# leekwoon/nav-gym

Hardware: AMD Instinct MI355X
Metric: env steps/sec (whole node), 4096 envs x 1081-beam lidar (higher is better)
Workload: dtype f32

## Files before the change

nav-gym_amd/csrc/kernels_step.hpp:

```cpp

struct StepShared {
    double rp[3];
    double old_rp[3];
    double act[2];
    float lx, ly, lth;
    int steps_now;
    double cT, sT;
    int i0, j0;
    int nseg, ndisc;
    int rescan;
    int respawn;
    float t1;
    float r_all;
    unsigned long long step_key;
    unsigned long long rescan_key;
    int next_chunk;
    int park_count, park_next;
    int pair_done;
    int term;
    int vote;
    double lin_step;
    float march_lim;
    double wave_ratio[kMaxWaves];
};
#ifndef NAVSIM_STEP_CONSTS_LDS
#define NAVSIM_STEP_CONSTS_LDS 1
#endif
#ifndef NAVSIM_STEP_VOTE_LDS
#define NAVSIM_STEP_VOTE_LDS 1
#endif
__device__ __forceinline__ double scan_lin_step(const navsim_config& c, const StepShared& sh) {
    if constexpr (NAVSIM_STEP_CONSTS_LDS) return sh.lin_step;
    else return nv::linspace_step(c);
}
__device__ __forceinline__ float scan_march_limit(const navsim_config& c, const StepShared& sh) {
    if constexpr (NAVSIM_STEP_CONSTS_LDS) return sh.march_lim;
    else return march_limit(c.map_h, c.map_w, c.range_max, c.resolution);
}
__device__ __forceinline__ void step_consts_publish(const navsim_config& c, StepShared& sh, int which) {
    const double num = which ? c.range_max : c.angle_last - c.angle_min;
    const double den = which ? c.resolution : (double)(c.n_beams - 1);
    const double q = num / den;
    if (which) {
        const float full = (float)((long long)c.map_h * c.map_w);
        const float lim = (float)(floor(q) + 4.0);
        sh.march_lim = lim < full ? lim : full;
    } else {
        sh.lin_step = (c.n_beams > 1) ? q : 0.0;
    }
}
struct PedShared {
    double *ax, *ay, *avx, *avy;
    float (*seg)[4];
    float (*disc)[2];
    float* info;
};
__host__ __device__ inline size_t ped_lds_bytes(int N) { return (size_t)144 * N + 32; }
__host__ __device__ inline size_t ped_pair_bytes(int N) { return ((size_t)(N * (N - 1) / 2 + N) * sizeof(double2) + 15) & ~(size_t)15; }
__device__ __forceinline__ PedShared ped_lds_carve(char* base, int N) {
    PedShared ps;
    double* d = (double*)base;
    ps.ax = d; ps.ay = d + (N + 1); ps.avx = d + 2 * (N + 1); ps.avy = d + 3 * (N + 1);
    float* f = (float*)(d + 4 * (N + 1));
    ps.seg = (float(*)[4])f;
    ps.disc = (float(*)[2])(f + 16 * N);
    ps.info = f + 20 * N;
    return ps;
}
struct Prims { const float (*seg)[4]; const float (*disc)[2]; float* info; };

template <int BLOCK>
__device__ __forceinline__ void finish_beams(const navsim_config& c, const StepShared& sh, const Prims pr,
                                             const double* __restrict__ tab, const float2* __restrict__ dir,
                                             const float* __restrict__ rng, float* __restrict__ rng_rw,
                                             const float* __restrict__ thr, const float* __restrict__ dthr,
                                             float* __restrict__ obs_row, int n_hist, float noise_std,
                                             uint64_t noise_key, uint64_t genv, int& crash, int& discomfort);

__device__ __forceinline__ void sfm_pair(const navsim_config& c, double xi, double yi, double vxi, double vyi,
                                         double xj, double yj, double vxj, double vyj, double& fx, double& fy) {
    fx = 0.0; fy = 0.0;
    double dxx = xj - xi, dyy = yj - yi;
    double dist = sqrt(dxx * dxx + dyy * dyy);
    if (dist < 1e-9) return;
    double ddx = dxx / dist, ddy = dyy / dist;
    double ivx = c.sfm_lambda * (vxi - vxj) + ddx;
    double ivy = c.sfm_lambda * (vyi - vyj) + ddy;
    double il = sqrt(ivx * ivx + ivy * ivy);
    if (il < 1e-9) return;
    double idx = ivx / il, idy = ivy / il;
    double theta = nv::atan2_(idx * ddy - idy * ddx, idx * ddx + idy * ddy);
    double Bq = c.sfm_gamma * il;
    double a1 = c.sfm_n_prime * Bq * theta;
    double a2 = c.sfm_n * Bq * theta;
    double fv = -nv::exp_neg(-dist / Bq - a1 * a1);
    double sgn = (theta > 0.0) ? 1.0 : ((theta < 0.0) ? -1.0 : 0.0);
    double fa = -sgn * nv::exp_neg(-dist / Bq - a2 * a2);
    fx = fv * idx + fa * (-idy);
    fy = fv * idy + fa * idx;
}

template <typename T>
__device__ __forceinline__ T& at_off32(T* base, int idx) {
    return *(T*)((char*)base + (unsigned)idx * (unsigned)sizeof(T));
}

__device__ __forceinline__ bool beam_dir_fast(double lin, double lth, double ct, double st, double cT, double sT,
                                              float& heading, float& dx, float& dy) {
    const double ang = lin + lth;
    heading = (float)ang;
    if constexpr (nv::kDirTwoSum) {
        const double bb = ang - lin;
        const double eps = (lin - (ang - bb)) + (lth - bb);
        const double delta = ((double)heading - ang) + eps;
        return nv::beam_dir_from_table(ct, st, cT, sT, delta, dx, dy);
    } else {
        const double delta = (double)heading - ang;
        const unsigned mag = (unsigned)__double2hiint(ang) & 0x7FFFFFFFu;
        return nv::beam_dir_from_table(ct, st, cT, sT, delta, dx, dy) & (mag < nv::kDirHi64);
    }
}
__device__ __forceinline__ void beam_dir_k(const navsim_config& c, const double* __restrict__ tab, int k,
                                           double step, double lth, double cT, double sT,
                                           float& dx, float& dy) {
#ifdef NAVSIM_DIAG_CHEAP_DIR
    { float h = (float)c.angle_min + (float)k * (float)step + (float)lth; dx = __cosf(h); dy = __sinf(h); return; }
#endif
    const double last = (c.n_beams == 1) ? c.angle_min : c.angle_last;
    const double lin = (k == c.n_beams - 1) ? last : (double)k * step + c.angle_min;
    float heading = (float)(lin + lth);
    bool fast = false;
    if (tab) {
        const double2 cs = at_off32((const double2*)tab, k);
        fast = beam_dir_fast(lin, lth, cs.x, cs.y, cT, sT, heading, dx, dy);
    }
    if (!fast) nv::beam_dir(heading, dx, dy);
}

template <int RULE, typename Field>
__device__ __forceinline__ void first_probe(const Field& field, int map_h, int map_w, int i0, int j0, float max_range,
                                            float& t1, float& r_all) {
    t1 = 0.0f; r_all = -1.0f;
    if (i0 >= map_w || j0 >= map_h) { r_all = max_range; return; }
    typename Field::raw_t raw0 = field.load(i0, j0);
    if (field.occupied(raw0)) { r_all = 0.0f; return; }
    t1 = march_step<RULE>(field.decode(raw0, i0, j0));
    if (!(t1 < max_range)) r_all = max_range;
}

constexpr float kPrimAllBeams = 1.0e30f;
template <int BLOCK> __device__ __forceinline__ int block_threads() { return BLOCK ? BLOCK : (int)blockDim.x; }
template <int BLOCK>
__device__ __forceinline__ void prim_in_range(int nprim, int nseg, float lx, float ly, float rcull, const Prims pr,
                                              float stepf, float beta0) {
    const float kTwoPiF = 6.2831853f;
    for (int p = (int)threadIdx.x; p < nprim; p += block_threads<BLOCK>()) {
        bool skip;
        float ac = 0.0f, w = 0.0f;
        bool full = (stepf <= 0.0f);
        if (p < nseg) {
            float ux = pr.seg[p][0] - lx, uy = pr.seg[p][1] - ly, vx = pr.seg[p][2] - lx, vy = pr.seg[p][3] - ly;
            skip = sqrtf(ux * ux + uy * uy) - sqrtf((vx - ux) * (vx - ux) + (vy - uy) * (vy - uy)) > rcull;
            float b1 = atan2f(uy, ux), b2 = atan2f(vy, vx);
            float d = b2 - b1;
            d -= kTwoPiF * floorf(d / kTwoPiF + 0.5f);
            ac = b1 + 0.5f * d;
            w = 0.5f * fabsf(d);
            if (fabsf(d) > 3.0f || ux * ux + uy * uy < 1e-6f || vx * vx + vy * vy < 1e-6f) full = true;
        } else {
            float ux = pr.disc[p - nseg][0] - lx, uy = pr.disc[p - nseg][1] - ly;
            float dist = sqrtf(ux * ux + uy * uy);
            skip = dist - nv::kLegRadius > rcull;
            if (dist <= nv::kLegRadius * 1.05f) full = true;
            else { ac = atan2f(uy, ux); w = asinf(fminf(1.0f, nv::kLegRadius / dist)); }
        }
        float rel = ac - beta0;
        rel -= kTwoPiF * floorf(rel / kTwoPiF + 0.5f);
// ... 706 lines not shown
    *peds_before = before;
    __syncthreads();
    return rank;
}

#ifndef NAVSIM_INSTALL_UNROLL
#define NAVSIM_INSTALL_UNROLL 8
#endif
struct StepInstallBig { char* dst; const char* src; size_t bytes; };
struct StepInstall {
    navsim_state stage;
    const float* stage_obs;
    uint8_t* mark;
    const long long* ready;
    uint8_t* late_next;
    const uint8_t* late_prev;
    int lone;
    uint8_t* late;
    StepInstallBig big[5];
};
__device__ __forceinline__ void stage_request(int64_t* stage_episode, uint8_t* mark, int e, int64_t ep) {
    __hip_atomic_store(&stage_episode[e], ep, __ATOMIC_RELAXED, __HIP_MEMORY_SCOPE_AGENT);
    __threadfence();
    atomicOr((unsigned*)(mark + (e & ~3)), 1u << (8 * (e & 3)));
}
__device__ __forceinline__ long long stage_ready(const long long* ready, int e) {
    return __hip_atomic_load(&ready[e], __ATOMIC_ACQUIRE, __HIP_MEMORY_SCOPE_AGENT);
}
__device__ __forceinline__ void install_publish(const StepInstall& in, const navsim_state& live, int e) {
    __syncthreads();
    if (threadIdx.x == 0) {
        __threadfence();
        stage_request(in.stage.episode, in.mark, e, live.episode[e] + 1);
    }
}
template <int BLOCK>
__device__ __forceinline__ void install_arena(const navsim_config& c, const navsim_state& live, const navsim_step_io& io,
                                              const StepInstall& in, const int e, float* __restrict__ obs_row) {
    const int tid = threadIdx.x;
    const bool by_slot = live.map_slot && in.stage.map_slot;
    if (by_slot && tid == 0) {
        const int32_t a = live.map_slot[e], b = in.stage.map_slot[e];
        live.map_slot[e] = b; in.stage.map_slot[e] = a;
    }
    for (int k = 0; k < 5 && !by_slot; ++k) {
        if (!in.big[k].dst) continue;
        const size_t bytes = in.big[k].bytes;
        const char* src = in.big[k].src + (size_t)e * bytes;
        char* dst = in.big[k].dst + (size_t)e * bytes;
        if ((((size_t)(uintptr_t)src | (size_t)(uintptr_t)dst | bytes) & 15) == 0) {
            const size_t n16 = bytes / 16;
            size_t i = tid;
#ifndef NAVSIM_DIAG_INSTALL_NO_BIG
            constexpr int U = NAVSIM_INSTALL_UNROLL;
            for (; i + (U - 1) * BLOCK < n16; i += U * BLOCK) {
                typedef unsigned int u32x4 __attribute__((ext_vector_type(4)));
                u32x4 v[U];
#pragma unroll
                for (int u = 0; u < U; ++u) v[u] = __builtin_nontemporal_load((const u32x4*)src + i + u * BLOCK);
#pragma unroll
                for (int u = 0; u < U; ++u) ((u32x4*)dst)[i + u * BLOCK] = v[u];
            }
            for (; i < n16; i += BLOCK) ((uint4*)dst)[i] = ((const uint4*)src)[i];
#endif
        } else {
            for (size_t i = tid; i < bytes; i += BLOCK) dst[i] = src[i];
        }
    }
    const navsim_state& stage = in.stage;
    const int N = c.max_peds, K = c.n_spawn, P = c.max_waypoints, D = c.n_scan_stack * c.n_beams + NAVSIM_OBS_TAIL;
    const bool peds = c.ped_model != NAVSIM_PED_NONE;
#define NAVSIM_ROW_LOAD(name, dstp, srcp, cnt) \
    const size_t n_##name = ((dstp) && (srcp)) ? (size_t)(cnt) : 0; \
    auto v_##name = (srcp)[tid < (int)n_##name ? (size_t)e * n_##name + tid : 0];
#define NAVSIM_ROW_STORE(name, dstp, srcp) \
    if (tid < (int)n_##name) (dstp)[(size_t)e * n_##name + tid] = v_##name; \
    for (size_t i = (size_t)tid + BLOCK; i < n_##name; i += BLOCK) (dstp)[(size_t)e * n_##name + i] = (srcp)[(size_t)e * n_##name + i];
#define NAVSIM_ROW_SRC(p) ((p) ? (p) : (decltype(p))live.steps)
    NAVSIM_ROW_LOAD(noise, live.scan_noise_std, NAVSIM_ROW_SRC(stage.scan_noise_std), 1)
    NAVSIM_ROW_LOAD(pose, live.robot_pose, NAVSIM_ROW_SRC(stage.robot_pose), 3)
    NAVSIM_ROW_LOAD(goal, live.robot_goal, NAVSIM_ROW_SRC(stage.robot_goal), 2)
    NAVSIM_ROW_LOAD(pact, live.prev_action, NAVSIM_ROW_SRC(stage.prev_action), 2)
    NAVSIM_ROW_LOAD(ppose, live.prev_pose, NAVSIM_ROW_SRC(stage.prev_pose), 3)
    NAVSIM_ROW_LOAD(nhist, live.n_hist, NAVSIM_ROW_SRC(stage.n_hist), 1)
    NAVSIM_ROW_LOAD(steps, live.steps, NAVSIM_ROW_SRC(stage.steps), 1)
    NAVSIM_ROW_LOAD(spose, live.spawn_pose, NAVSIM_ROW_SRC(stage.spawn_pose), (size_t)K * 3)
    NAVSIM_ROW_LOAD(sgoal, live.spawn_goal, NAVSIM_ROW_SRC(stage.spawn_goal), (size_t)K * 2)
    NAVSIM_ROW_LOAD(npeds, peds ? live.n_peds : nullptr, NAVSIM_ROW_SRC(stage.n_peds), 1)
    NAVSIM_ROW_LOAD(ppos, peds ? live.ped_pose : nullptr, NAVSIM_ROW_SRC(stage.ped_pose), (size_t)N * 3)
    NAVSIM_ROW_LOAD(pvel, peds ? live.ped_vel : nullptr, NAVSIM_ROW_SRC(stage.ped_vel), (size_t)N * 2)
    NAVSIM_ROW_LOAD(pyaw, peds ? live.ped_prev_yaw : nullptr, NAVSIM_ROW_SRC(stage.ped_prev_yaw), N)
    NAVSIM_ROW_LOAD(pdist, peds ? live.ped_dist : nullptr, NAVSIM_ROW_SRC(stage.ped_dist), (size_t)N * 3)
    NAVSIM_ROW_LOAD(pvpref, peds ? (double*)live.ped_v_pref : nullptr, NAVSIM_ROW_SRC(stage.ped_v_pref), N)
    NAVSIM_ROW_LOAD(plegs, peds ? (uint8_t*)live.ped_has_legs : nullptr, NAVSIM_ROW_SRC(stage.ped_has_legs), N)
    NAVSIM_ROW_LOAD(pwp, peds ? live.ped_waypoints : nullptr, NAVSIM_ROW_SRC(stage.ped_waypoints), (size_t)N * P * 2)
    NAVSIM_ROW_LOAD(pnwp, peds ? live.ped_n_waypoints : nullptr, NAVSIM_ROW_SRC(stage.ped_n_waypoints), N)
    NAVSIM_ROW_LOAD(phead, peds ? live.ped_wp_head : nullptr, NAVSIM_ROW_SRC(stage.ped_wp_head), N)
    NAVSIM_ROW_LOAD(pgoal, peds ? live.ped_goal : nullptr, NAVSIM_ROW_SRC(stage.ped_goal), (size_t)N * 2)
    NAVSIM_ROW_LOAD(obs, obs_row - (size_t)e * D, in.stage_obs, D)
    NAVSIM_ROW_STORE(noise, live.scan_noise_std, stage.scan_noise_std)
    NAVSIM_ROW_STORE(pose, live.robot_pose, stage.robot_pose)
    NAVSIM_ROW_STORE(goal, live.robot_goal, stage.robot_goal)
    NAVSIM_ROW_STORE(pact, live.prev_action, stage.prev_action)
    NAVSIM_ROW_STORE(ppose, live.prev_pose, stage.prev_pose)
    NAVSIM_ROW_STORE(nhist, live.n_hist, stage.n_hist)
    NAVSIM_ROW_STORE(steps, live.steps, stage.steps)
    NAVSIM_ROW_STORE(spose, (double*)live.spawn_pose, stage.spawn_pose)
    NAVSIM_ROW_STORE(sgoal, (double*)live.spawn_goal, stage.spawn_goal)
    NAVSIM_ROW_STORE(npeds, live.n_peds, stage.n_peds)
    NAVSIM_ROW_STORE(ppos, live.ped_pose, stage.ped_pose)
    NAVSIM_ROW_STORE(pvel, live.ped_vel, stage.ped_vel)
    NAVSIM_ROW_STORE(pyaw, live.ped_prev_yaw, stage.ped_prev_yaw)
    NAVSIM_ROW_STORE(pdist, live.ped_dist, stage.ped_dist)
    NAVSIM_ROW_STORE(pvpref, (double*)live.ped_v_pref, stage.ped_v_pref)
    NAVSIM_ROW_STORE(plegs, (uint8_t*)live.ped_has_legs, stage.ped_has_legs)
    NAVSIM_ROW_STORE(pwp, live.ped_waypoints, stage.ped_waypoints)
    NAVSIM_ROW_STORE(pnwp, live.ped_n_waypoints, stage.ped_n_waypoints)
    NAVSIM_ROW_STORE(phead, live.ped_wp_head, stage.ped_wp_head)
    NAVSIM_ROW_STORE(pgoal, live.ped_goal, stage.ped_goal)
    NAVSIM_ROW_STORE(obs, obs_row - (size_t)e * D, in.stage_obs)
#undef NAVSIM_ROW_LOAD
#undef NAVSIM_ROW_STORE
#undef NAVSIM_ROW_SRC
    if (tid == 0) {
        if (io.achieved_goal) { io.achieved_goal[2 * e] = (float)stage.robot_pose[3 * (size_t)e]; io.achieved_goal[2 * e + 1] = (float)stage.robot_pose[3 * (size_t)e + 1]; }
        if (io.desired_goal) { io.desired_goal[2 * e] = (float)stage.robot_goal[2 * (size_t)e]; io.desired_goal[2 * e + 1] = (float)stage.robot_goal[2 * (size_t)e + 1]; }
        if (live.ped_due) live.ped_due[e] = 0ull;
    }
}

template <int BLOCK, bool PEDS, typename Field, int RULE, int RECT, bool PINL, bool INSTALL = false, bool FEAT = true>
__device__ __forceinline__ void step_arena(const navsim_config& c, const navsim_state& st, const navsim_step_io& io, const int e,
                                           int reset_only, const int peds_done, const uint8_t* __restrict__ reset_mask,
                                           unsigned dyn_lds_bytes, int park_lanes, unsigned rect_lds_offset,
                                           const StepInstall* in = nullptr, const int base_prio = 0) {
    __shared__ StepShared sh;
    extern __shared__ __attribute__((aligned(16))) char dyn_lds_all[];
    char* dyn_lds = dyn_lds_all + (RECT == 2 ? rect_lds_offset : 0u);
    PedShared ps = {};
    if constexpr (PEDS) ps = ped_lds_carve(dyn_lds + ((dyn_lds_bytes + 15u) & ~15u), c.max_peds);
    const Prims prims = {ps.seg, ps.disc, ps.info};
    const int tid = threadIdx.x;
    constexpr int kMarchPrio = (BLOCK == 256 && !PEDS) ? 2 : 0;
    __builtin_amdgcn_s_setprio(3);
    unsigned long long t_begin = 0;
    if (st.arena_cost && tid == 0) t_begin = __builtin_amdgcn_s_memrealtime();
    const int B = c.n_beams, S = c.n_scan_stack, N = c.max_peds, D = S * B + 7;
    const double dt = c.time_step;
    const uint64_t genv = (uint64_t)(c.env_index_base + e);
    const int ms = INSTALL ? map_slot_of(c, st, e) : (c.shared_field ? 0 : e);
    const Field field(st.field, st.field_overflow, ms, c.map_h, c.map_w);
    const uint4* rects = RECT ? (const uint4*)st.rect_table + (size_t)ms * rect_tiles_per_map(c.map_h, c.map_w)
                              : nullptr;
    if constexpr (RECT == 2) {
        const size_t row_bytes = rect_index_row_bytes(c.map_h, c.map_w);
        const uint4* src = (const uint4*)((const char*)st.rect_index + (size_t)ms * row_bytes);
        uint4* tab_lds = (uint4*)dyn_lds_all;
        for (int i = threadIdx.x; i < (int)(row_bytes / 16); i += BLOCK) tab_lds[i] = src[i];
        rects = tab_lds;
    }
    float* obs_row = io.obs + (size_t)e * D;
    const float* obs_prev = io.obs_prev ? io.obs_prev + (size_t)e * D : nullptr;
    double* rp_g = st.robot_pose + 3 * (size_t)e;
    double* goal_g = st.robot_goal + 2 * (size_t)e;
    double* pa_g = st.prev_action + 2 * (size_t)e;
    double* pv_g = st.prev_pose + 3 * (size_t)e;

    constexpr bool kFeat = PEDS || FEAT;
    const bool pending = kFeat && !reset_only && io.reset_mask && io.reset_mask[e] != 0;
    if (pending) {
        reset_only = 1;
        if (tid == 0) {
            io.reward[e] = 0.0; io.done[e] = 0; io.is_success[e] = 0.0f; io.is_crash[e] = 0.0f; io.distance[e] = 0.0;
            if (c.max_episode_steps > 0 && io.truncated) io.truncated[e] = 0;
            if (st.ped_due) st.ped_due[e] = 0ull;
        }
        if (c.defer_reset_scan) return;
        if constexpr (INSTALL && BLOCK >= 256 && RULE == NAVSIM_MARCH_F32) {
            if (in->lone && in->ready) {
                if (tid == 0) {
                    const bool lng = c.regen_min_steps <= 0 || st.done_steps[e] >= c.regen_min_steps;
                    const bool rdy = stage_ready(in->ready, e) == (long long)st.episode[e];
                    sh.respawn = lng ? (rdy ? 3 : 5) : 0;
                    if (!(lng && rdy)) stage_request(in->stage.episode, in->mark, e, st.episode[e] + 1);
                    if (st.counters) {
                        atomicAdd(&st.counters[lng ? (rdy ? NAVSIM_COUNTER_REGEN_SERVED : NAVSIM_COUNTER_REGEN_LATE) : NAVSIM_COUNTER_REGEN_SHORT], 1ull);
                        if (lng && !rdy) atomicAdd(&st.counters[NAVSIM_COUNTER_REGEN_SERVED], 1ull);
                    }
                }
                __syncthreads();
                const int verdict = sh.respawn;
                __syncthreads();
                if (verdict == 3) {
                    install_arena<BLOCK>(c, st, io, *in, e, obs_row);
                    install_publish(*in, st, e);
                    return;
                }
                if (verdict == 5) {
                    regen_lone<Field, BLOCK>(c, st, e);
                    if constexpr (RECT == 2) {
                        const size_t row_bytes = rect_index_row_bytes(c.map_h, c.map_w);
                        const uint4* src = (const uint4*)((const char*)st.rect_index + (size_t)ms * row_bytes);
                        uint4* tab_lds = (uint4*)dyn_lds_all;
                        for (int i = threadIdx.x; i < (int)(row_bytes / 16); i += BLOCK) tab_lds[i] = src[i];
                    }
                }
            }
        }
    }
    if (reset_only && reset_mask && !reset_mask[e]) {
        if (obs_prev && obs_prev != obs_row)
            for (int k = tid; k < D; k += BLOCK) obs_row[k] = obs_prev[k];
        return;
    }

    int n = (!PEDS || c.ped_model == NAVSIM_PED_NONE) ? 0 : st.n_peds[e];
    n = n > N ? N : n;
    const float noise_std = (c.add_scan_noise && st.scan_noise_std) ? st.scan_noise_std[e] : 0.0f;

    NAVSIM_STAMP(0);
    double pp[3] = {0.0, 0.0, 0.0};
    double pvel[2] = {0.0, 0.0};
    const bool is_ped = PEDS && tid < n;
    const size_t pq = (size_t)e * N + (is_ped ? tid : 0);
    const bool ped_advance = PEDS && PINL && !reset_only && !peds_done;
    int ped_head = 0, ped_nw = 1;
    if constexpr (PEDS) {
        if (tid < 64) {
            if (is_ped) {
                pp[0] = st.ped_pose[pq * 3]; pp[1] = st.ped_pose[pq * 3 + 1]; pp[2] = st.ped_pose[pq * 3 + 2];
                pvel[0] = st.ped_vel[pq * 2]; pvel[1] = st.ped_vel[pq * 2 + 1];
            }
            if constexpr (PINL) {
                if (ped_advance) ped_head = ped_stage_wave(c, st, n, tid, is_ped, pq, rp_g, pa_g[0], ps, pp, pvel, ped_nw);
            }
        }
    }
    constexpr int kPhase0Thread = (PEDS && BLOCK > 64) ? 64 : 0;
    const int l0 = tid - kPhase0Thread;
    if (l0 >= 0 && l0 < (NAVSIM_STEP_CONSTS_LDS ? 5 : 3)) {
        const double th_old = rp_g[2];
        double a0 = 0.0, a1 = 0.0;
        if (!reset_only) {
            a0 = io.action[2 * e]; a1 = io.action[2 * e + 1];
            if (c.action_kind == NAVSIM_ACTION_WHEELS) {
                const double wl = a0, wr = a1;
                a0 = c.wheel_radius * (wl + wr) * 0.5;
                a1 = c.wheel_radius * (wr - wl) / c.wheel_track;
            }
            if (c.clamp_action) {
                a0 = a0 < c.linvel_lo ? c.linvel_lo : (a0 > c.linvel_hi ? c.linvel_hi : a0);
                a1 = a1 < c.rotvel_lo ? c.rotvel_lo : (a1 > c.rotvel_hi ? c.rotvel_hi : a1);
            }
            if (c.min_turning_radius > 0.0) {
                double lim = fabs(a1) * c.min_turning_radius;
                if (a0 >= 0.0) a0 = (a0 > lim) ? a0 : lim;
                else           a0 = (a0 < -lim) ? a0 : -lim;
            }
        }
        const double th = th_old + a1 * dt;
        const double th_new = reset_only ? th_old : nv::mod_2pi(th);
        const float lth = (float)th_new;
        const double ang = (l0 == 0) ? th_old : ((l0 == 1) ? th : (double)lth);
        double sn, cs;
        nv::sincos(ang, sn, cs);
        const int w0 = kPhase0Thread & 63;
        const double s0 = __shfl(sn, w0), c0 = __shfl(cs, w0), s1 = __shfl(sn, w0 + 1), c1 = __shfl(cs, w0 + 1);
        const double sT = __shfl(sn, w0 + 2), cT = __shfl(cs, w0 + 2);
        if (NAVSIM_STEP_CONSTS_LDS && l0 >= 3) step_consts_publish(c, sh, l0 - 3);
        if (l0 == 0) {
            sh.old_rp[0] = rp_g[0]; sh.old_rp[1] = rp_g[1]; sh.old_rp[2] = th_old;
            sh.nseg = 0; sh.ndisc = 0; sh.rescan = 0; sh.respawn = 0; sh.term = 0;
            if constexpr (INSTALL) {
                if (pending && !in->lone) {
                    if (in->late) in->late[e] = 0;
                    if (in->late_next) in->late_next[e] = 0;
                    if (in->late_prev && in->late_prev[e]) {
                        sh.respawn = 4;
                        stage_request(in->stage.episode, in->mark, e, st.episode[e] + 1);
                        if (st.counters) atomicAdd(&st.counters[NAVSIM_COUNTER_REGEN_LATE], 1ull);
                    } else if (in->ready) {
                        const bool lng = c.regen_min_steps <= 0 || st.done_steps[e] >= c.regen_min_steps;
                        const bool rdy = stage_ready(in->ready, e) == (long long)st.episode[e];
                        if (lng && rdy) sh.respawn = 3;
                        else {
                            if (lng && in->late) in->late[e] = 1;
                            stage_request(in->stage.episode, in->mark, e, st.episode[e] + 1);
                        }
                        if (st.counters)
                            atomicAdd(&st.counters[lng ? (rdy ? NAVSIM_COUNTER_REGEN_SERVED : NAVSIM_COUNTER_REGEN_LATE) : NAVSIM_COUNTER_REGEN_SHORT], 1ull);
                    }
                }
            }
            if (!reset_only) {
                const int64_t steps_now = st.steps[e] + 1;
                st.steps[e] = steps_now;
                sh.steps_now = (int)steps_now;
                sh.act[0] = a0; sh.act[1] = a1;
                double p[3] = {sh.old_rp[0], sh.old_rp[1], sh.old_rp[2]};
                nv::set_vel_with(p, a0, a1, dt, c.axle_offset, s0, c0, s1, c1, nullptr);
                sh.rp[0] = p[0]; sh.rp[1] = p[1]; sh.rp[2] = p[2];
            } else {
                sh.rp[0] = sh.old_rp[0]; sh.rp[1] = sh.old_rp[1]; sh.rp[2] = sh.old_rp[2];
            }
            sh.lx = (float)sh.rp[0]; sh.ly = (float)sh.rp[1]; sh.lth = (float)sh.rp[2];
            nv::xy_to_ij_f32(sh.lx, sh.ly, c, sh.i0, sh.j0);
            sh.sT = sT; sh.cT = cT;
            first_probe<RULE>(field, c.map_h, c.map_w, sh.i0, sh.j0, (float)((long long)c.map_h * c.map_w), sh.t1, sh.r_all);
            sh.step_key = (unsigned long long)st.episode[e] * 0x100000000ULL +
                          (unsigned long long)(reset_only ? 0 : st.steps[e]) * 2ULL;
            sh.rescan_key = sh.step_key + 1;
            sh.next_chunk = 0; sh.park_count = 0; sh.park_next = 0; sh.pair_done = 0; sh.vote = 0;
        }
    }
    __syncthreads();
    if constexpr (INSTALL) {
        if (pending && sh.respawn == 3) {
            install_arena<BLOCK>(c, st, io, *in, e, obs_row);
            install_publish(*in, st, e);
            return;
        }
        if (pending && sh.respawn == 4) return;
    }

    NAVSIM_STAMP(1);
    if constexpr (PEDS) {
        double2* pair = (double2*)(dyn_lds + ((dyn_lds_bytes + 15u) & ~15u) + ((ped_lds_bytes(N) + 15) & ~(size_t)15));
#ifdef NAVSIM_PAIR_SHARE_ALL
        constexpr int kPairWaves = (BLOCK >= NAVSIM_PAIR_SHARE_MIN_BLOCK) ? 4 : 1;
#else
        constexpr int kPairWaves = (INSTALL && BLOCK >= NAVSIM_PAIR_SHARE_MIN_BLOCK) ? 4 : 1;
#endif
        const bool pair_shared = PINL && kPairWaves > 1 && ped_advance && c.ped_model == NAVSIM_PED_SFM;
        if constexpr (PINL && kPairWaves > 1) {
            if (pair_shared && tid < kPairWaves * 64) ped_pair_share(c, ps, pair, n, tid, kPairWaves, &sh.pair_done);
        }
        if (tid < 64) {
            const int lane = tid;
            if constexpr (PINL) {
                if (ped_advance)
                    ped_advance_wave<Field>(c, st, field, e, n, lane, is_ped, pq, dt, genv, (uint64_t)st.steps[e], ps, pair,
                                            ped_head, ped_nw, pp, pvel, &sh.pair_done, pair_shared ? kPairWaves : 1);
            }
            if (reset_only && is_ped) {
                st.ped_dist[pq * 3] = 0.0; st.ped_dist[pq * 3 + 1] = 0.0; st.ped_dist[pq * 3 + 2] = 0.0;
                st.ped_prev_yaw[pq] = nv::wrap_pi(pp[2]);
            }
            if (is_ped) {
                float dist3[3];
                if (reset_only) { dist3[0] = dist3[1] = dist3[2] = 0.0f; }
                else { dist3[0] = (float)st.ped_dist[pq * 3]; dist3[1] = (float)st.ped_dist[pq * 3 + 1];
                       dist3[2] = (float)st.ped_dist[pq * 3 + 2]; }
                if (st.ped_has_legs[pq] && c.lidar_legs) {
                    float cc[4];
                    nv::leg_centres((float)pp[0], (float)pp[1], (float)pp[2], dist3[0], dist3[1], dist3[2], cc);
                    int q = atomicAdd(&sh.ndisc, 2);
                    ps.disc[q][0] = cc[0]; ps.disc[q][1] = cc[1];
                    ps.disc[q + 1][0] = cc[2]; ps.disc[q + 1][1] = cc[3];
                } else {
                    const double fpx[4] = {0.22, -0.22, -0.22, 0.22};
                    const double fpy[4] = {0.19, 0.19, -0.19, -0.19};
                    double s, cs;
                    nv::sincos(pp[2], s, cs);
                    float vx[4], vy[4];
#pragma unroll
                    for (int v = 0; v < 4; ++v) {
                        vx[v] = (float)((cs * fpx[v] - s * fpy[v]) + pp[0]);
                        vy[v] = (float)((s * fpx[v] + cs * fpy[v]) + pp[1]);
                    }
                    int q = atomicAdd(&sh.nseg, 4);
#pragma unroll
                    for (int v = 0; v < 4; ++v) {
                        int w = (v + 1) & 3;
                        ps.seg[q + v][0] = vx[v]; ps.seg[q + v][1] = vy[v];
                        ps.seg[q + v][2] = vx[w]; ps.seg[q + v][3] = vy[w];
                    }
                }
            }
            wave_lds_sync();
            prims_prepare<64>(c, sh, prims);
        }
    }

    NAVSIM_STAMP(2);
    if (kMarchPrio == 2 || base_prio == 2) __builtin_amdgcn_s_setprio(2);
    else if (base_prio == 1) __builtin_amdgcn_s_setprio(1);
    else __builtin_amdgcn_s_setprio(0);
    int n_hist = reset_only ? 0 : st.n_hist[e];
    int crash = 0, discomfort = 0;
    const uint64_t step_key = sh.step_key;
    float4* park = (float4*)dyn_lds;
    char* scan_lds = dyn_lds + park_lds_bytes(B, park_lanes, PEDS);
    float2* dir_lds = (float2*)scan_lds;
    float* rng_lds = (float*)(scan_lds + sizeof(float2) * (size_t)B);
    scan_beams_pred<BLOCK, Field, PEDS, RULE, RECT>(c, sh, field, rects, st.beam_table, prims, dir_lds, rng_lds, park, park_lanes, st.scan_threshold,
                                                         st.scan_discomfort, obs_row, n_hist, noise_std, step_key, genv, crash, discomfort, false);

    NAVSIM_STAMP(3);
    bool restart_next = false;
    if (!reset_only) {
        vote_flags<BLOCK, PEDS>(sh, crash, discomfort);
        double rmin = 1.0e300;
        if (discomfort && !crash) {
            for (int k = tid; k < B; k += BLOCK)
            {
                double ratio = nv::discomfort_ratio((double)obs_row[(size_t)(S - 1) * B + k],
                                                    st.scan_threshold[k], st.scan_discomfort[k]);
                rmin = ratio < rmin ? ratio : rmin;
            }
            rmin = wave_min_f64(rmin);
            if ((tid & 63) == 0) sh.wave_ratio[tid >> 6] = rmin;
            __syncthreads();
        }
        NAVSIM_STAMP(4);
        if (tid == 0) {
            if (discomfort && !crash)
                for (int w = 1; w < (BLOCK + 63) / 64; ++w) rmin = sh.wave_ratio[w] < rmin ? sh.wave_ratio[w] : rmin;
            double prev_xy[2] = {pv_g[0], pv_g[1]};
            double pose[2] = {sh.rp[0], sh.rp[1]};
            double vel[2] = {pa_g[0], pa_g[1]};
            double goal[2] = {goal_g[0], goal_g[1]};
            nv::RewardOut o = nv::reward_scalar(c, prev_xy, pose, vel, goal, crash != 0, discomfort != 0, rmin);
            if constexpr (kFeat) {
                if (c.max_episode_steps > 0) {
                    const bool trunc = !o.done && sh.steps_now >= c.max_episode_steps;
                    if (io.truncated) io.truncated[e] = (uint8_t)trunc;
                    if (trunc) o.done = 1;
                }
            }
            io.reward[e] = o.reward;
            io.done[e] = (uint8_t)o.done;
            if constexpr (INSTALL) { if (in->late) in->late[e] = 0; if (in->late_next) in->late_next[e] = 0; }
            io.is_success[e] = o.success;
            io.is_crash[e] = o.crash;
            io.distance[e] = o.distance;
            const bool restart = o.done && c.auto_reset != NAVSIM_AUTORESET_NONE && c.n_spawn > 0;
            if (restart && c.auto_reset == NAVSIM_AUTORESET_SAME_STEP) {
                if (kFeat && io.final_obs) {
                    const bool crashed = o.crash != 0.0f;
                    const double tx = crashed ? pv_g[0] : sh.rp[0], ty = crashed ? pv_g[1] : sh.rp[1];
                    const double tyaw = nv::wrap_pi(crashed ? pv_g[2] : sh.rp[2]);
                    float* ft = io.final_obs + (size_t)e * D + (size_t)S * B;
                    ft[0] = (float)pv_g[0]; ft[1] = (float)pv_g[1];
                    ft[2] = (float)tx; ft[3] = (float)ty;
                    ft[4] = (float)pa_g[0]; ft[5] = (float)pa_g[1];
                    ft[6] = (float)tyaw;
                    if (io.final_goals) {
                        float* fg = io.final_goals + 4 * (size_t)e;
                        fg[0] = (float)tx; fg[1] = (float)ty; fg[2] = (float)goal_g[0]; fg[3] = (float)goal_g[1];
                    }
                    sh.term = crashed ? 2 : 1;
                }
                uint64_t h = nv::hash4(c.seed, genv, (uint64_t)st.episode[e], 0x5eedULL);
                int idx = (int)(h % (uint64_t)c.n_spawn);
                const double* sp = st.spawn_pose + ((size_t)e * c.n_spawn + idx) * 3;
                const double* sg = st.spawn_goal + ((size_t)e * c.n_spawn + idx) * 2;
                sh.rp[0] = sp[0]; sh.rp[1] = sp[1]; sh.rp[2] = sp[2];
                goal_g[0] = sg[0]; goal_g[1] = sg[1];
#ifndef NAVSIM_DIAG_NO_DONE_STEPS
                if (st.done_steps) st.done_steps[e] = sh.steps_now;
#endif
                st.episode[e] += 1;
                st.steps[e] = 0;
                sh.rescan_key = (unsigned long long)st.episode[e] * 0x100000000ULL;
                sh.respawn = 1; sh.rescan = c.defer_reset_scan ? 0 : 1;
                if constexpr (INSTALL) if (in->ready) {
                    const bool lng = c.regen_min_steps <= 0 || st.done_steps[e] >= c.regen_min_steps;
                    const bool rdy = stage_ready(in->ready, e) == (long long)st.episode[e];
                    if (lng && rdy) { sh.respawn = 3; sh.rescan = 0; }
                    else if (lng && in->late) in->late[e] = 1;
                    if (st.counters)
                        atomicAdd(&st.counters[lng ? (rdy ? NAVSIM_COUNTER_REGEN_SERVED : NAVSIM_COUNTER_REGEN_LATE) : NAVSIM_COUNTER_REGEN_SHORT], 1ull);
                    if (!(lng && rdy)) stage_request(in->stage.episode, in->mark, e, st.episode[e] + 1);
                }
            } else {
                restart_next = kFeat && restart;
                if (o.crash != 0.0f) {
                    sh.rp[0] = pv_g[0]; sh.rp[1] = pv_g[1]; sh.rp[2] = pv_g[2];
                    sh.rescan = 1;
                }
            }
#ifdef NAVSIM_DIAG_NO_RESCAN
            sh.rescan = 0;
#endif
            if constexpr (!kFeat) {
                if (sh.rescan) {
                    sh.next_chunk = 0; sh.park_count = 0; sh.park_next = 0;
                    sh.lx = (float)sh.rp[0]; sh.ly = (float)sh.rp[1]; sh.lth = (float)sh.rp[2];
                    nv::xy_to_ij_f32(sh.lx, sh.ly, c, sh.i0, sh.j0);
                    nv::sincos((double)sh.lth, sh.sT, sh.cT);
                    first_probe<RULE>(field, c.map_h, c.map_w, sh.i0, sh.j0, (float)((long long)c.map_h * c.map_w), sh.t1, sh.r_all);
                }
            }
        }
        __syncthreads();
        if constexpr (!kFeat) {
            if (sh.rescan) {
                if (sh.respawn) n_hist = 0;
                int c2, d2;
                scan_beams_pred<BLOCK, Field, PEDS, RULE, RECT>(c, sh, field, rects, st.beam_table, prims, dir_lds, rng_lds, park, park_lanes, st.scan_threshold,
                                                                     st.scan_discomfort, obs_row, n_hist, noise_std, sh.rescan_key, genv, c2, d2);
            }
        } else {
            float* final_row = io.final_obs ? io.final_obs + (size_t)e * D : nullptr;
            const int term = sh.term;
            if (term == 1) {
                for (int j = 0; j < S; ++j) {
                    const bool old = j < S - 1 && S - 1 - j <= n_hist;
                    for (int k = tid; k < B; k += BLOCK)
                        final_row[(size_t)j * B + k] = old ? obs_prev[(size_t)(j + 1) * B + k] : obs_row[(size_t)(S - 1) * B + k];
                }
                __syncthreads();
            }
            for (int pass = (term == 2) ? 0 : 1; pass < 2; ++pass) {
                if (pass == 1 && !sh.rescan) break;
                if (tid == 0) {
                    const double* at = (pass == 0) ? pv_g : sh.rp;
                    sh.next_chunk = 0; sh.park_count = 0; sh.park_next = 0;
                    sh.lx = (float)at[0]; sh.ly = (float)at[1]; sh.lth = (float)at[2];
                    nv::xy_to_ij_f32(sh.lx, sh.ly, c, sh.i0, sh.j0);
                    nv::sincos((double)sh.lth, sh.sT, sh.cT);
                    first_probe<RULE>(field, c.map_h, c.map_w, sh.i0, sh.j0, (float)((long long)c.map_h * c.map_w), sh.t1, sh.r_all);
                }
                __syncthreads();
                if (pass == 1 && sh.respawn) n_hist = 0;
                int c2, d2;
                scan_beams_pred<BLOCK, Field, PEDS, RULE, RECT>(c, sh, field, rects, st.beam_table, prims, dir_lds, rng_lds, park, park_lanes, st.scan_threshold,
                                                                     st.scan_discomfort, pass == 0 ? final_row : obs_row, n_hist, noise_std,
                                                                     pass == 0 ? step_key + 1 : sh.rescan_key, genv, c2, d2);
                if (pass == 0) {
                    for (int j = 0; j < S - 1; ++j)
                        if (S - 1 - j <= n_hist)
                            for (int k = tid; k < B; k += BLOCK) final_row[(size_t)j * B + k] = obs_prev[(size_t)(j + 1) * B + k];
                    __syncthreads();
                }
            }
        }
    }

    NAVSIM_STAMP(5);
    if (kMarchPrio != 0 && base_prio < kMarchPrio) {
        if (base_prio == 1) __builtin_amdgcn_s_setprio(1);
        else __builtin_amdgcn_s_setprio(0);
    }
    const bool fresh = reset_only || sh.respawn;
    if (!fresh && obs_prev) {
        for (int j = 0; j < S - 1; ++j)
            if (S - 1 - j <= n_hist)
                for (int k = tid; k < B; k += BLOCK) obs_row[(size_t)j * B + k] = obs_prev[(size_t)(j + 1) * B + k];
    }
    if (tid == 0) {
        float* tail = obs_row + (size_t)S * B;
        double yaw = nv::wrap_pi(sh.rp[2]);
        double pxy0 = fresh ? sh.rp[0] : pv_g[0];
        double pxy1 = fresh ? sh.rp[1] : pv_g[1];
        double v0 = fresh ? 0.0 : pa_g[0], v1 = fresh ? 0.0 : pa_g[1];
        tail[0] = (float)pxy0; tail[1] = (float)pxy1;
        tail[2] = (float)sh.rp[0]; tail[3] = (float)sh.rp[1];
        tail[4] = (float)v0; tail[5] = (float)v1;
        tail[6] = (float)yaw;
        if (io.achieved_goal) { io.achieved_goal[2 * e] = (float)sh.rp[0]; io.achieved_goal[2 * e + 1] = (float)sh.rp[1]; }
        if (io.desired_goal) { io.desired_goal[2 * e] = (float)goal_g[0]; io.desired_goal[2 * e + 1] = (float)goal_g[1]; }
        rp_g[0] = sh.rp[0]; rp_g[1] = sh.rp[1]; rp_g[2] = sh.rp[2];
        if (fresh) { pa_g[0] = 0.0; pa_g[1] = 0.0; st.n_hist[e] = (S - 1 < 1) ? S - 1 : 1; }
        else       { pa_g[0] = sh.act[0]; pa_g[1] = sh.act[1]; st.n_hist[e] = (n_hist + 1 < S - 1) ? n_hist + 1 : S - 1; }
        if (reset_only) st.steps[e] = 0;
        pv_g[0] = sh.rp[0]; pv_g[1] = sh.rp[1]; pv_g[2] = yaw;
        if (restart_next) {
            uint64_t h = nv::hash4(c.seed, genv, (uint64_t)st.episode[e], 0x5eedULL);
            int idx = (int)(h % (uint64_t)c.n_spawn);
            const double* sp = st.spawn_pose + ((size_t)e * c.n_spawn + idx) * 3;
            const double* sg = st.spawn_goal + ((size_t)e * c.n_spawn + idx) * 2;
            rp_g[0] = sp[0]; rp_g[1] = sp[1]; rp_g[2] = sp[2];
            goal_g[0] = sg[0]; goal_g[1] = sg[1];
            if (st.done_steps) st.done_steps[e] = sh.steps_now;
            st.episode[e] += 1;
            st.steps[e] = 0;
            if constexpr (INSTALL) {
                if (in->late_next && in->ready) {
                    const bool lng = c.regen_min_steps <= 0 || sh.steps_now >= c.regen_min_steps;
                    const bool rdy = stage_ready(in->ready, e) == (long long)st.episode[e];
                    in->late_next[e] = (lng && !rdy) ? 1 : 0;
                }
            }
        }
        if (st.arena_cost && !reset_only)
            st.arena_cost[e] = (uint32_t)(__builtin_amdgcn_s_memrealtime() - t_begin);
    }
    NAVSIM_STAMP(6);
    if constexpr (INSTALL) {
        __syncthreads();
        if (sh.respawn == 3) {
            install_arena<BLOCK>(c, st, io, *in, e, obs_row);
            install_publish(*in, st, e);
        }
        NAVSIM_STAMP(7);
    }
}

constexpr int kOrderBuckets = 1024;
struct OrderLds {
    unsigned long long sum;
    unsigned max, pad;
    unsigned wave_tot[16];
    unsigned hist[kOrderBuckets];
};
constexpr size_t kOrderLdsBytes = sizeof(OrderLds);
struct OrderBuckets {
    unsigned long long m;
    float scale;
    __device__ __forceinline__ OrderBuckets(unsigned max, unsigned long long sum, int n) {
        const unsigned long long cap = 4ull * (sum / (unsigned long long)n) + 1ull;
        m = max < cap ? max : cap;
        scale = (float)(kOrderBuckets - 1) / (float)m;
    }
    __device__ __forceinline__ int operator()(unsigned cst) const {
        const unsigned long long cc = cst < m ? cst : m;
        const int b = (int)((float)cc * scale);
        return kOrderBuckets - 1 - (b > kOrderBuckets - 1 ? kOrderBuckets - 1 : b);
    }
};
template <int BLOCK>
__device__ __forceinline__ void order_scan(OrderLds& s) {
    constexpr int K = kOrderBuckets / BLOCK, WAVES = BLOCK / 64;
    static_assert(K >= 1 && K * BLOCK == kOrderBuckets && WAVES <= 16, "one workgroup of 64 .. 1024 threads");
    const int tid = threadIdx.x, lane = tid & 63;
    unsigned mine = 0;
    for (int k = 0; k < K; ++k) mine += s.hist[tid * K + k];
    unsigned incl = mine;
    for (int off = 1; off < 64; off <<= 1) {
        const unsigned v = __shfl_up(incl, off, 64);
        if (lane >= off) incl += v;
    }
    unsigned run = incl - mine;
    if constexpr (WAVES > 1) {
        if (lane == 63) s.wave_tot[tid >> 6] = incl;
        __syncthreads();
        if (tid < 64) {
            const unsigned t = tid < WAVES ? s.wave_tot[tid] : 0u;
            unsigned ti = t;
            for (int off = 1; off < WAVES; off <<= 1) {
                const unsigned v = __shfl_up(ti, off, 64);
                if (tid >= off) ti += v;
            }
            if (tid < WAVES) s.wave_tot[tid] = ti - t;
        }
        __syncthreads();
        run += s.wave_tot[tid >> 6];
    }
    for (int k = 0; k < K; ++k) {
        const unsigned h = s.hist[tid * K + k];
        s.hist[tid * K + k] = run;
        run += h;
    }
    __syncthreads();
}
template <int BLOCK>
__device__ __forceinline__ void launch_order_sort(const uint32_t* __restrict__ cost, int32_t* __restrict__ order, int n, OrderLds& s) {
    const int tid = threadIdx.x;
    for (int b = tid; b < kOrderBuckets; b += BLOCK) s.hist[b] = 0;
    if (tid == 0) { s.max = 1; s.sum = 0; }
    __syncthreads();
    unsigned mx = 0;
    unsigned long long sm = 0;
    for (int e = tid; e < n; e += BLOCK) { mx = cost[e] > mx ? cost[e] : mx; sm += cost[e]; }
    atomicMax(&s.max, mx);
    atomicAdd(&s.sum, sm);
    __syncthreads();
    const OrderBuckets bucket(s.max, s.sum, n);
    for (int e = tid; e < n; e += BLOCK) atomicAdd(&s.hist[bucket(cost[e])], 1u);
    __syncthreads();
    order_scan<BLOCK>(s);
    for (int e = tid; e < n; e += BLOCK) order[atomicAdd(&s.hist[bucket(cost[e])], 1u)] = e;
}
__global__ __launch_bounds__(1024) void launch_order_kernel(const uint32_t* __restrict__ cost, int32_t* __restrict__ order,
                                                            int n) {
    __shared__ OrderLds s;
    launch_order_sort<1024>(cost, order, n, s);
}

#ifndef NAVSIM_KARG_VIEW
#define NAVSIM_KARG_VIEW 1
#endif
struct StepKernargs { navsim_config c; navsim_state st; navsim_step_io io; };
struct StepInstallKernargs { navsim_config c; navsim_state st; navsim_step_io io; StepInstall in; };
#if NAVSIM_KARG_VIEW
#define NAVSIM_KERNARGS(View, ...) const View& ka = *(const View*)__builtin_amdgcn_kernarg_segment_ptr()
#else
#define NAVSIM_KERNARGS(View, ...) const View ka = {__VA_ARGS__}
#endif
constexpr int kStepWordResetOnly = 1, kStepWordPedsDoneBit = 1, kStepWordPartShift = 2, kStepWordPartMask = 3, kStepWordSortBit = 4;
constexpr int kStepPartReplan = 3;
template <int BLOCK, bool PEDS, typename Field, int RULE, int RECT, bool PINL, bool FEAT = true>
#ifndef NAVSIM_PEDS_WAVES_MIN
#define NAVSIM_PEDS_WAVES_MIN 5
#endif
#ifndef NAVSIM_NOPEDS_WAVES_MIN
#define NAVSIM_NOPEDS_WAVES_MIN 8
#endif
__global__ __launch_bounds__(BLOCK) __attribute__((amdgpu_waves_per_eu((PEDS && PINL && RECT == 2 && BLOCK == 256) ? NAVSIM_PEDS_WAVES_MIN : (!PEDS ? NAVSIM_NOPEDS_WAVES_MIN : 8), 8)))
void navsim_step_kernel(navsim_config c_, navsim_state st_,
                                                            navsim_step_io io_, int reset_only,
                                                            const uint8_t* __restrict__ reset_mask,
                                                            unsigned dyn_lds_bytes, int park_lanes, unsigned rect_lds_offset,
                                                            const uint32_t* __restrict__ sort_cost, int32_t* __restrict__ sort_order) {
    NAVSIM_KERNARGS(StepKernargs, c_, st_, io_);
    const navsim_config& c = ka.c; const navsim_state& st = ka.st; const navsim_step_io& io = ka.io;
    const int peds_done = (reset_only >> kStepWordPedsDoneBit) & 1;
    const int part = (reset_only >> kStepWordPartShift) & kStepWordPartMask;
    const int front = (reset_only >> kStepWordSortBit) & 1;
    reset_only &= kStepWordResetOnly;
    if (front && blockIdx.x == 0) {
        extern __shared__ __attribute__((aligned(16))) char dyn_lds_all[];
        __builtin_amdgcn_s_setprio(3);
        launch_order_sort<BLOCK>(sort_cost, sort_order, c.n_envs, *(OrderLds*)dyn_lds_all);
// ... 96 lines not shown
```

Before: 55.29 million.

## Prefetch per-env step scalars alongside batched rect-index LDS copy and cache in LDS

Loads all per-env scalar state (pose, action, steps, episode, n_hist, noise std, prev pose, goal, prev action) into registers early, issuing them between the batched loads and stores of the rect-index row copy into LDS. Those values are then published to shared memory so later phases (reward, tail write, rescan) read LDS instead of re-reading global memory. The LDS copy is restructured to issue four 16-byte loads per thread before storing. The intent is to hide serial global-load latency at kernel start, at the cost of extra registers and LDS and some added complexity in template-gated code paths.

```diff
diff --git a/nav-gym_amd/csrc/kernels_step.hpp b/nav-gym_amd/csrc/kernels_step.hpp
--- a/nav-gym_amd/csrc/kernels_step.hpp
+++ b/nav-gym_amd/csrc/kernels_step.hpp
@@ -22,7 +22,79 @@
     double lin_step;
     float march_lim;
     double wave_ratio[kMaxWaves];
+    double prev_pose[3], goal[2], prev_action[2];
+    long long steps64;
+    int n_hist;
+    float noise_std;
 };
+#ifndef NAVSIM_HEAD_ROW_BATCH
+#define NAVSIM_HEAD_ROW_BATCH 1
+#endif
+#ifndef NAVSIM_HEAD_SCALARS
+#define NAVSIM_HEAD_SCALARS 1
+#endif
+#ifndef NAVSIM_HEAD_ALL_LANES
+#define NAVSIM_HEAD_ALL_LANES 1
+#endif
+#ifndef NAVSIM_HEAD_EVERYWHERE
+#define NAVSIM_HEAD_EVERYWHERE 0
+#endif
+#ifndef NAVSIM_HEAD_TAIL
+#define NAVSIM_HEAD_TAIL 1
+#endif
+constexpr int kRowBatch = 4;
+template <int BLOCK>
+__device__ __forceinline__ void row_batch_load(uint4 (&v)[kRowBatch], const uint4* __restrict__ src, int base, int n16) {
+#pragma unroll
+    for (int k = 0; k < kRowBatch; ++k) {
+        const int i = base + k * BLOCK;
+        v[k] = src[i < n16 ? i : base];
+    }
+}
+template <int BLOCK>
+__device__ __forceinline__ void row_batch_store(const uint4 (&v)[kRowBatch], uint4* dst, int base, int n16) {
+#pragma unroll
+    for (int k = 0; k < kRowBatch; ++k) {
+        const int i = base + k * BLOCK;
+        dst[i < n16 ? i : base] = v[k];
+    }
+}
+template <int BLOCK, bool BATCH = true>
+__device__ __forceinline__ void row_copy(uint4* dst, const uint4* __restrict__ src, int n16, int first = 0) {
+    if constexpr (NAVSIM_HEAD_ROW_BATCH && BATCH) {
+        for (int base = (int)threadIdx.x + first * kRowBatch * BLOCK; base < n16; base += kRowBatch * BLOCK) {
+            uint4 v[kRowBatch];
+            row_batch_load<BLOCK>(v, src, base, n16);
+            row_batch_store<BLOCK>(v, dst, base, n16);
+        }
+    } else {
+        for (int i = threadIdx.x; i < n16; i += BLOCK) dst[i] = src[i];
+    }
+}
+struct StepHead {
+    double rp[3], act[2], prev_pose[3], goal[2], prev_action[2];
+    long long steps;
+    unsigned episode_lo;
+    int n_hist;
+    float noise_std;
+};
+__device__ __forceinline__ void step_head_load(StepHead& h, const navsim_config& c, const navsim_state& st, const navsim_step_io& io,
+                                               int e, bool with_action) {
+    const double* rp_g = st.robot_pose + 3 * (size_t)e;
+    const double* pv_g = st.prev_pose + 3 * (size_t)e;
+    const double* goal_g = st.robot_goal + 2 * (size_t)e;
+    const double* pa_g = st.prev_action + 2 * (size_t)e;
+    h.rp[0] = rp_g[0]; h.rp[1] = rp_g[1]; h.rp[2] = rp_g[2];
+    h.act[0] = 0.0; h.act[1] = 0.0;
+    if (with_action) { h.act[0] = io.action[2 * e]; h.act[1] = io.action[2 * e + 1]; }
+    h.steps = st.steps[e];
+    h.episode_lo = *(const unsigned*)(st.episode + e);
+    h.n_hist = st.n_hist[e];
+    h.noise_std = (c.add_scan_noise && st.scan_noise_std) ? st.scan_noise_std[e] : 0.0f;
+    h.prev_pose[0] = pv_g[0]; h.prev_pose[1] = pv_g[1]; h.prev_pose[2] = pv_g[2];
+    h.goal[0] = goal_g[0]; h.goal[1] = goal_g[1];
+    h.prev_action[0] = pa_g[0]; h.prev_action[1] = pa_g[1];
+}
 #ifndef NAVSIM_STEP_CONSTS_LDS
 #define NAVSIM_STEP_CONSTS_LDS 1
 #endif
@@ -1035,12 +1107,35 @@
     const Field field(st.field, st.field_overflow, ms, c.map_h, c.map_w);
     const uint4* rects = RECT ? (const uint4*)st.rect_table + (size_t)ms * rect_tiles_per_map(c.map_h, c.map_w)
                               : nullptr;
+    constexpr int kPhase0Thread = (PEDS && BLOCK > 64) ? 64 : 0;
+    constexpr bool kNewHead = NAVSIM_HEAD_EVERYWHERE != 0 ||
+                              !(INSTALL || (PEDS && BLOCK >= 1024) || (!PEDS && FEAT) || (PEDS && !PINL));
+    constexpr bool kHead = NAVSIM_HEAD_SCALARS != 0 && kNewHead, kTail = NAVSIM_HEAD_TAIL != 0 && kNewHead;
+    const int l0 = tid - kPhase0Thread;
+    const bool phase0_lane = l0 >= 0 && l0 < (NAVSIM_STEP_CONSTS_LDS ? 5 : 3);
+    const bool with_action = !reset_only;
+    StepHead hd;
     if constexpr (RECT == 2) {
         const size_t row_bytes = rect_index_row_bytes(c.map_h, c.map_w);
         const uint4* src = (const uint4*)((const char*)st.rect_index + (size_t)ms * row_bytes);
         uint4* tab_lds = (uint4*)dyn_lds_all;
-        for (int i = threadIdx.x; i < (int)(row_bytes / 16); i += BLOCK) tab_lds[i] = src[i];
+        const int n16 = (int)(row_bytes / 16);
+        if constexpr (NAVSIM_HEAD_ROW_BATCH && kHead && !INSTALL) {
+            uint4 v[kRowBatch];
+            const int base = tid < n16 ? tid : 0;
+            row_batch_load<BLOCK>(v, src, base, n16);
+            if (NAVSIM_HEAD_ALL_LANES || phase0_lane) step_head_load(hd, c, st, io, e, with_action);
+            row_batch_store<BLOCK>(v, tab_lds, base, n16);
+            row_copy<BLOCK>(tab_lds, src, n16, 1);
+        } else {
+            if constexpr (kHead && !INSTALL) {
+                if (NAVSIM_HEAD_ALL_LANES || phase0_lane) step_head_load(hd, c, st, io, e, with_action);
+            }
+            row_copy<BLOCK, kNewHead>(tab_lds, src, n16);
+        }
         rects = tab_lds;
+    } else if constexpr (kHead && !INSTALL) {
+        if (NAVSIM_HEAD_ALL_LANES || phase0_lane) step_head_load(hd, c, st, io, e, with_action);
     }
     float* obs_row = io.obs + (size_t)e * D;
     const float* obs_prev = io.obs_prev ? io.obs_prev + (size_t)e * D : nullptr;
@@ -1048,6 +1143,9 @@
     double* goal_g = st.robot_goal + 2 * (size_t)e;
     double* pa_g = st.prev_action + 2 * (size_t)e;
     double* pv_g = st.prev_pose + 3 * (size_t)e;
+    const double* pv_r = kTail ? sh.prev_pose : pv_g;
+    const double* goal_r = kTail ? sh.goal : goal_g;
+    const double* pa_r = kTail ? sh.prev_action : pa_g;
 
     constexpr bool kFeat = PEDS || FEAT;
     const bool pending = kFeat && !reset_only && io.reset_mask && io.reset_mask[e] != 0;
@@ -1084,8 +1182,7 @@
                     if constexpr (RECT == 2) {
                         const size_t row_bytes = rect_index_row_bytes(c.map_h, c.map_w);
                         const uint4* src = (const uint4*)((const char*)st.rect_index + (size_t)ms * row_bytes);
-                        uint4* tab_lds = (uint4*)dyn_lds_all;
-                        for (int i = threadIdx.x; i < (int)(row_bytes / 16); i += BLOCK) tab_lds[i] = src[i];
+                        row_copy<BLOCK, kNewHead>((uint4*)dyn_lds_all, src, (int)(row_bytes / 16));
                     }
                 }
             }
@@ -1099,7 +1196,8 @@
 
     int n = (!PEDS || c.ped_model == NAVSIM_PED_NONE) ? 0 : st.n_peds[e];
     n = n > N ? N : n;
-    const float noise_std = (c.add_scan_noise && st.scan_noise_std) ? st.scan_noise_std[e] : 0.0f;
+    float noise_std = 0.0f;
+    if constexpr (!kHead) noise_std = (c.add_scan_noise && st.scan_noise_std) ? st.scan_noise_std[e] : 0.0f;
 
     NAVSIM_STAMP(0);
     double pp[3] = {0.0, 0.0, 0.0};
@@ -1119,13 +1217,13 @@
             }
         }
     }
-    constexpr int kPhase0Thread = (PEDS && BLOCK > 64) ? 64 : 0;
-    const int l0 = tid - kPhase0Thread;
-    if (l0 >= 0 && l0 < (NAVSIM_STEP_CONSTS_LDS ? 5 : 3)) {
-        const double th_old = rp_g[2];
+    if (phase0_lane) {
+        if constexpr (kHead && INSTALL) step_head_load(hd, c, st, io, e, !reset_only);
+        const double th_old = kHead ? hd.rp[2] : rp_g[2];
         double a0 = 0.0, a1 = 0.0;
         if (!reset_only) {
-            a0 = io.action[2 * e]; a1 = io.action[2 * e + 1];
+            if constexpr (kHead) { a0 = hd.act[0]; a1 = hd.act[1]; }
+            else { a0 = io.action[2 * e]; a1 = io.action[2 * e + 1]; }
             if (c.action_kind == NAVSIM_ACTION_WHEELS) {
                 const double wl = a0, wr = a1;
                 a0 = c.wheel_radius * (wl + wr) * 0.5;
@@ -1152,7 +1250,14 @@
         const double sT = __shfl(sn, w0 + 2), cT = __shfl(cs, w0 + 2);
         if (NAVSIM_STEP_CONSTS_LDS && l0 >= 3) step_consts_publish(c, sh, l0 - 3);
         if (l0 == 0) {
-            sh.old_rp[0] = rp_g[0]; sh.old_rp[1] = rp_g[1]; sh.old_rp[2] = th_old;
+            sh.old_rp[0] = kHead ? hd.rp[0] : rp_g[0]; sh.old_rp[1] = kHead ? hd.rp[1] : rp_g[1]; sh.old_rp[2] = th_old;
+            if constexpr (kHead) { sh.n_hist = hd.n_hist; sh.noise_std = hd.noise_std; }
+            if constexpr (kTail) {
+                sh.prev_pose[0] = kHead ? hd.prev_pose[0] : pv_g[0]; sh.prev_pose[1] = kHead ? hd.prev_pose[1] : pv_g[1];
+                sh.prev_pose[2] = kHead ? hd.prev_pose[2] : pv_g[2];
+                sh.goal[0] = kHead ? hd.goal[0] : goal_g[0]; sh.goal[1] = kHead ? hd.goal[1] : goal_g[1];
+                sh.prev_action[0] = kHead ? hd.prev_action[0] : pa_g[0]; sh.prev_action[1] = kHead ? hd.prev_action[1] : pa_g[1];
+            }
             sh.nseg = 0; sh.ndisc = 0; sh.rescan = 0; sh.respawn = 0; sh.term = 0;
             if constexpr (INSTALL) {
                 if (pending && !in->lone) {
@@ -1175,10 +1280,12 @@
                     }
                 }
             }
+            int64_t key_steps = 0;
             if (!reset_only) {
-                const int64_t steps_now = st.steps[e] + 1;
+                const int64_t steps_now = (kHead ? (int64_t)hd.steps : st.steps[e]) + 1;
                 st.steps[e] = steps_now;
                 sh.steps_now = (int)steps_now;
+                if constexpr (kHead) { sh.steps64 = steps_now; key_steps = steps_now; }
                 sh.act[0] = a0; sh.act[1] = a1;
                 double p[3] = {sh.old_rp[0], sh.old_rp[1], sh.old_rp[2]};
                 nv::set_vel_with(p, a0, a1, dt, c.axle_offset, s0, c0, s1, c1, nullptr);
@@ -1190,8 +1297,11 @@
             nv::xy_to_ij_f32(sh.lx, sh.ly, c, sh.i0, sh.j0);
             sh.sT = sT; sh.cT = cT;
             first_probe<RULE>(field, c.map_h, c.map_w, sh.i0, sh.j0, (float)((long long)c.map_h * c.map_w), sh.t1, sh.r_all);
-            sh.step_key = (unsigned long long)st.episode[e] * 0x100000000ULL +
-                          (unsigned long long)(reset_only ? 0 : st.steps[e]) * 2ULL;
+            if constexpr (kHead)
+                sh.step_key = (unsigned long long)hd.episode_lo * 0x100000000ULL + (unsigned long long)key_steps * 2ULL;
+            else
+                sh.step_key = (unsigned long long)st.episode[e] * 0x100000000ULL +
+                              (unsigned long long)(reset_only ? 0 : st.steps[e]) * 2ULL;
             sh.rescan_key = sh.step_key + 1;
             sh.next_chunk = 0; sh.park_count = 0; sh.park_next = 0; sh.pair_done = 0; sh.vote = 0;
         }
@@ -1222,7 +1332,7 @@
             const int lane = tid;
             if constexpr (PINL) {
                 if (ped_advance)
-                    ped_advance_wave<Field>(c, st, field, e, n, lane, is_ped, pq, dt, genv, (uint64_t)st.steps[e], ps, pair,
+                    ped_advance_wave<Field>(c, st, field, e, n, lane, is_ped, pq, dt, genv, kHead ? (uint64_t)sh.steps64 : (uint64_t)st.steps[e], ps, pair,
                                             ped_head, ped_nw, pp, pvel, &sh.pair_done, pair_shared ? kPairWaves : 1);
             }
             if (reset_only && is_ped) {
@@ -1269,7 +1379,8 @@
     if (kMarchPrio == 2 || base_prio == 2) __builtin_amdgcn_s_setprio(2);
     else if (base_prio == 1) __builtin_amdgcn_s_setprio(1);
     else __builtin_amdgcn_s_setprio(0);
-    int n_hist = reset_only ? 0 : st.n_hist[e];
+    int n_hist = reset_only ? 0 : (kHead ? sh.n_hist : st.n_hist[e]);
+    if constexpr (kHead) noise_std = sh.noise_std;
     int crash = 0, discomfort = 0;
     const uint64_t step_key = sh.step_key;
     float4* park = (float4*)dyn_lds;
@@ -1299,10 +1410,10 @@
         if (tid == 0) {
             if (discomfort && !crash)
                 for (int w = 1; w < (BLOCK + 63) / 64; ++w) rmin = sh.wave_ratio[w] < rmin ? sh.wave_ratio[w] : rmin;
-            double prev_xy[2] = {pv_g[0], pv_g[1]};
+            double prev_xy[2] = {pv_r[0], pv_r[1]};
             double pose[2] = {sh.rp[0], sh.rp[1]};
-            double vel[2] = {pa_g[0], pa_g[1]};
-            double goal[2] = {goal_g[0], goal_g[1]};
+            double vel[2] = {pa_r[0], pa_r[1]};
+            double goal[2] = {goal_r[0], goal_r[1]};
             nv::RewardOut o = nv::reward_scalar(c, prev_xy, pose, vel, goal, crash != 0, discomfort != 0, rmin);
             if constexpr (kFeat) {
                 if (c.max_episode_steps > 0) {
@@ -1321,16 +1432,16 @@
             if (restart && c.auto_reset == NAVSIM_AUTORESET_SAME_STEP) {
                 if (kFeat && io.final_obs) {
                     const bool crashed = o.crash != 0.0f;
-                    const double tx = crashed ? pv_g[0] : sh.rp[0], ty = crashed ? pv_g[1] : sh.rp[1];
-                    const double tyaw = nv::wrap_pi(crashed ? pv_g[2] : sh.rp[2]);
+                    const double tx = crashed ? pv_r[0] : sh.rp[0], ty = crashed ? pv_r[1] : sh.rp[1];
+                    const double tyaw = nv::wrap_pi(crashed ? pv_r[2] : sh.rp[2]);
                     float* ft = io.final_obs + (size_t)e * D + (size_t)S * B;
-                    ft[0] = (float)pv_g[0]; ft[1] = (float)pv_g[1];
+                    ft[0] = (float)pv_r[0]; ft[1] = (float)pv_r[1];
                     ft[2] = (float)tx; ft[3] = (float)ty;
-                    ft[4] = (float)pa_g[0]; ft[5] = (float)pa_g[1];
+                    ft[4] = (float)pa_r[0]; ft[5] = (float)pa_r[1];
                     ft[6] = (float)tyaw;
                     if (io.final_goals) {
                         float* fg = io.final_goals + 4 * (size_t)e;
-                        fg[0] = (float)tx; fg[1] = (float)ty; fg[2] = (float)goal_g[0]; fg[3] = (float)goal_g[1];
+                        fg[0] = (float)tx; fg[1] = (float)ty; fg[2] = (float)goal_r[0]; fg[3] = (float)goal_r[1];
                     }
                     sh.term = crashed ? 2 : 1;
                 }
@@ -1340,6 +1451,7 @@
                 const double* sg = st.spawn_goal + ((size_t)e * c.n_spawn + idx) * 2;
                 sh.rp[0] = sp[0]; sh.rp[1] = sp[1]; sh.rp[2] = sp[2];
                 goal_g[0] = sg[0]; goal_g[1] = sg[1];
+                if constexpr (kTail) { sh.goal[0] = sg[0]; sh.goal[1] = sg[1]; }
 #ifndef NAVSIM_DIAG_NO_DONE_STEPS
                 if (st.done_steps) st.done_steps[e] = sh.steps_now;
 #endif
@@ -1359,7 +1471,7 @@
             } else {
                 restart_next = kFeat && restart;
                 if (o.crash != 0.0f) {
-                    sh.rp[0] = pv_g[0]; sh.rp[1] = pv_g[1]; sh.rp[2] = pv_g[2];
+                    sh.rp[0] = pv_r[0]; sh.rp[1] = pv_r[1]; sh.rp[2] = pv_r[2];
                     sh.rescan = 1;
                 }
             }
@@ -1398,7 +1510,7 @@
             for (int pass = (term == 2) ? 0 : 1; pass < 2; ++pass) {
                 if (pass == 1 && !sh.rescan) break;
                 if (tid == 0) {
-                    const double* at = (pass == 0) ? pv_g : sh.rp;
+                    const double* at = (pass == 0) ? pv_r : sh.rp;
                     sh.next_chunk = 0; sh.park_count = 0; sh.park_next = 0;
                     sh.lx = (float)at[0]; sh.ly = (float)at[1]; sh.lth = (float)at[2];
                     nv::xy_to_ij_f32(sh.lx, sh.ly, c, sh.i0, sh.j0);
@@ -1435,15 +1547,15 @@
     if (tid == 0) {
         float* tail = obs_row + (size_t)S * B;
         double yaw = nv::wrap_pi(sh.rp[2]);
-        double pxy0 = fresh ? sh.rp[0] : pv_g[0];
-        double pxy1 = fresh ? sh.rp[1] : pv_g[1];
-        double v0 = fresh ? 0.0 : pa_g[0], v1 = fresh ? 0.0 : pa_g[1];
+        double pxy0 = fresh ? sh.rp[0] : pv_r[0];
+        double pxy1 = fresh ? sh.rp[1] : pv_r[1];
+        double v0 = fresh ? 0.0 : pa_r[0], v1 = fresh ? 0.0 : pa_r[1];
         tail[0] = (float)pxy0; tail[1] = (float)pxy1;
         tail[2] = (float)sh.rp[0]; tail[3] = (float)sh.rp[1];
         tail[4] = (float)v0; tail[5] = (float)v1;
         tail[6] = (float)yaw;
         if (io.achieved_goal) { io.achieved_goal[2 * e] = (float)sh.rp[0]; io.achieved_goal[2 * e + 1] = (float)sh.rp[1]; }
-        if (io.desired_goal) { io.desired_goal[2 * e] = (float)goal_g[0]; io.desired_goal[2 * e + 1] = (float)goal_g[1]; }
+        if (io.desired_goal) { io.desired_goal[2 * e] = (float)goal_r[0]; io.desired_goal[2 * e + 1] = (float)goal_r[1]; }
         rp_g[0] = sh.rp[0]; rp_g[1] = sh.rp[1]; rp_g[2] = sh.rp[2];
         if (fresh) { pa_g[0] = 0.0; pa_g[1] = 0.0; st.n_hist[e] = (S - 1 < 1) ? S - 1 : 1; }
         else       { pa_g[0] = sh.act[0]; pa_g[1] = sh.act[1]; st.n_hist[e] = (n_hist + 1 < S - 1) ? n_hist + 1 : S - 1; }
```

After: 57.91 million, median of 6. 1.05x the previous value.
